# 0xMiden/miden-vm

Measured on NVIDIA H100. Metric: trace cells/sec proved, higher is better.
Workload: dtype u64

## Files before the change

### miden-vm_b200/csrc/kernels.cuh

```cuda
#pragma once
#include "gl.cuh"
#include <cuda_runtime.h>

namespace mk {
using gl::u64;
using gl::u32;
using gl::E2;

static constexpr u32 MAX_RANKS = 8;
struct PeerPtrs { u64* p[MAX_RANKS]; };
enum PushMode : u32 { PUSH_LOCAL = 0, PUSH_OWNER = 1, PUSH_ALL = 2 };
struct PushDst { PeerPtrs pp; u32 rank, world, mode, owner_shift; };
inline PushDst local_dst(u64* p) { PushDst d{}; d.pp.p[0] = p; d.rank = 0; d.world = 1; d.mode = PUSH_LOCAL; d.owner_shift = 0; return d; }

void launch_barrier(const PeerPtrs& flags, u32 rank, u32 world, u64 epoch, u32* err, cudaStream_t st);
void launch_push(const u64* src, const PeerPtrs& dst, u32 rank, u32 world, size_t n, cudaStream_t st);

struct NttTables {
    u32 n, n1, n2, lo_bits;
    const u64* tw_n1;
    const u64* twi_n1;
    const u64* twi_n2;
    const u64* w_lo;
    const u64* w_hi;
    const u64* wi_lo;
    const u64* wi_hi;
};
struct PremulTables {
    const u64* tab_b;
    const u64* tab_c;
};

void launch_transpose_rm_to_cm(const u64* src_rm, u64* dst_cm, u32 n_rows, u32 width, u32* d_bad_flag, cudaStream_t st);
void launch_transpose_slice_push(const u64* src_slice, const PeerPtrs& dst_cm, const PeerPtrs& bad, u32 world, u32 row0, u32 n_rows_slice,
                                 u32 n_rows_total, u32 width, cudaStream_t st);
void launch_ingest_cm(const u64* src_cm, u64* dst_cm, size_t n, u32* d_bad_flag, cudaStream_t st);

void launch_intt(u64* cols, size_t col_stride, u32 n_cols, const NttTables& T, cudaStream_t st);

struct FwdItem { const u64* src; u64* dst; u32 base; u32 pad; };
void launch_fwd_ntt(const FwdItem* d_items, u32 n_items, const NttTables& T, const PremulTables& Pm, cudaStream_t st);

struct LeafMat { const u64* base; u32 width; u32 pad; };
struct LeafArgs { LeafMat m[8]; int n_mats; };
void launch_leaf_hash(const LeafArgs& a, u32 log_n, u32 log_blowup, const u64* prev_states, u32 prev_log_n,
                      u64* states_out, const PushDst* dig, u32 t0, u32 nt, cudaStream_t st, int perm = 0);
void launch_compress_layer(const u64* children, u64* parents, size_t n_parents, cudaStream_t st, int perm = 0);
void launch_fri_leaf_hash(const u64* evals , size_t rows, u32 log_arity, const PushDst& digests,
                          u32 log_b, u32 t0, u32 nt, cudaStream_t st, int perm = 0);
void launch_poseidon2_batch(u64* states, size_t n, cudaStream_t st);
void launch_compress_top(u64* tree, u32 d_from, u32 lg, u32 rank, int hash_kind, cudaStream_t st);
void launch_leaf_hash_b3(const LeafArgs& a, u32 log_n, u32 log_blowup, const u64* prev_states, u32 prev_log_n,
                         u64* states_out, const PushDst* dig, u32 t0, u32 nt, cudaStream_t st);
void launch_compress_layer_b3(const u64* children, u64* parents, size_t n_parents, cudaStream_t st);
void launch_fri_leaf_hash_b3(const u64* evals, size_t rows, u32 log_arity, const PushDst& digests, u32 log_b, u32 t0, u32 nt, cudaStream_t st);
void launch_grind_b3(const u32* d_input_words, u32 n_words, u32 bits, u64 start, u64 count, u64* d_result, cudaStream_t st);
void launch_leaf_hash_kk(const LeafArgs& a, u32 log_n, u32 log_blowup, const u64* prev_states, u32 prev_log_n,
                         u64* states_out, const PushDst* dig, u32 t0, u32 nt, cudaStream_t st);
void launch_compress_layer_kk(const u64* children, u64* parents, size_t n_parents, cudaStream_t st);
void launch_fri_leaf_hash_kk(const u64* evals, size_t rows, u32 log_arity, const PushDst& digests, u32 log_b, u32 t0, u32 nt, cudaStream_t st);
void launch_grind_kk(const u64* d_input_words, u32 n_words, u32 bits, u64 start, u64 count, u64* d_result, cudaStream_t st);

struct AirDev {
    const u32* code;
    const u64* consts;
    const u64* periodic;
    u32 n_instr, n_slots;
    u32 uses_selectors;
    u32 log_max_period, n_periodic;
};
struct ConstraintArgs {
    const u64* main_lde; u32 main_width;
    const u64* aux_lde; u32 aux_width_base;
    const u64* prep_lde;
    u32 log_n, log_blowup;
    AirDev air;
    const u64* publics;
    const u64* challenges;
    const u64* aux_values;
    E2 alpha, beta;
    const u64* acc_in; u32 acc_in_log_n;
    u64* acc_out;
    const NttTables* T;
    u32 t0, nt;
};
int launch_constraints(const ConstraintArgs& a, cudaStream_t st);

struct LogupArgs {
    const u64* main_cm;
    const u64* prep_cm;
    u32 log_n, n_cols;
    AirDev prog;
    const u64* publics; const u64* challenges;
    u64* aux_cm;
    u64* totals;
    u32* bad_flag;
};
int launch_logup_rows(const LogupArgs& a, cudaStream_t st);
void launch_ef_exclusive_scan(const u64* totals, size_t n, u64* acc0, u64* acc1, u64* final2, u64* scratch, cudaStream_t st);
static constexpr u32 LOGUP_MAX_COLS = 16;

static constexpr u32 REG_MAX = 4, REG_BLOCK = 128;
struct RegisterArgs {
    const u64* main_cm;
    const u64* prep_cm;
    u32 log_n, n_regs;
    u32 col0;
    AirDev prog;
    const u64* publics; const u64* challenges;
    u64* aux_cm;
    u64* scratch;
    u32* bad_flag;
};
size_t register_scratch_words(u32 log_n, u32 n_regs);
int launch_register_columns(const RegisterArgs& a, cudaStream_t st);

struct CheckArgs {
    const u64* main_cm;
    const u64* aux_cm;
    const u64* prep_cm;
    u32 log_n;
    AirDev prog;
    const u64* publics; const u64* challenges; const u64* aux_values;
    size_t row0, n_rows;
    unsigned long long* first;
    unsigned long long* failing_rows;
    u32 probe_k; u64* probe_value;
};
int launch_check_rows(const CheckArgs& a, cudaStream_t st);

static constexpr u32 CENSUS_SHARED_K = 256;
struct CensusArgs {
    const u64* main_cm; const u64* aux_cm; const u64* prep_cm;
    u32 log_n;
    AirDev prog;
    const u64* publics; const u64* challenges; const u64* aux_values;
    u32 n_cons;
    u32 instance;
    u32* row_count;
    unsigned long long* tally;
    unsigned long long* failing_rows;
    const u64* offsets;
    u64 max_failures;
    u64* failures;
    const u64* probes; size_t n_probes;
};
int launch_census_rows(const CensusArgs& a, cudaStream_t st);
int launch_census_list(const CensusArgs& a, cudaStream_t st);
void launch_count_exclusive_scan(const u32* counts, size_t n, u64* offsets, u64* total, u64* scratch, cudaStream_t st);

struct BalanceTable {
    u64* keys;
    u64* sums;
    unsigned long long* count;
    unsigned long long* first;
    u64 mask;
};
static constexpr u32 BALANCE_BOUNDARY = 0x100;
__host__ __device__ inline u64 balance_key(u32 inst, u64 row, u32 k) { return ((u64)inst << 48) | (row << 24) | k; }
static constexpr u32 BALANCE_MUTEX_MAX = 1024;
struct BalanceArgs {
    const u64* main_cm; u32 log_n;
    const u64* prep_cm;
    AirDev prog;
    const u64* publics; const u64* challenges;
    u32 instance, mode;
    const u32* mutex_pos; const u32* mutex_group; const u32* mutex_site; u32 n_mutex;
    BalanceTable t;
    unsigned long long* counters;
    u64* mutex_out;
    u64* contrib_out;
};
int launch_balance_rows(const BalanceArgs& a, cudaStream_t st);
void launch_balance_boundary(const BalanceTable& t, const u64* triples, u32 n, cudaStream_t st);
void launch_balance_finish(const BalanceTable& t, unsigned long long* counters, u64* out, cudaStream_t st);
void launch_balance_compare(const BalanceTable& a, const BalanceTable& b, unsigned long long* words, cudaStream_t st);

struct LookupFoldArgs {
    const u64* main_cm; u32 log_n, n_cols;
    const u64* prep_cm;
    AirDev prog;
    const u64* publics; const u64* challenges;
    const u32* marks;
    const u64* aux_cm;
    E2 final;
    u64* folds_out; u32 folds_cm;
    size_t row0, n_rows;
    unsigned long long* first;
    unsigned long long* failing_rows;
    unsigned long long* zero_u;
    u32 probe_col; u64* probe;
};
int launch_fold_rows(const LookupFoldArgs& a, cudaStream_t st);

static constexpr u32 FOLD_RECORD_WORDS = 11;
struct FoldCensusArgs {
    const u64* main_cm; u32 log_n, n_cols;
    const u64* prep_cm;
    AirDev prog;
    const u64* publics; const u64* challenges;
    const u32* marks;
    const u64* aux_cm;
    E2 final;
    u32 instance;
    u32* row_count;
    unsigned long long* tally;
    unsigned long long* failing_rows;
    const u64* offsets;
    u64 max_failures;
    u64* failures;
    const u64* probes; size_t n_probes;
};
int launch_fold_census_rows(const FoldCensusArgs& a, cudaStream_t st);
int launch_fold_census_list(const FoldCensusArgs& a, cudaStream_t st);

void launch_pow_bitrev(E2 y, u32 n, u64* wvec, u64* scratch, size_t p0, size_t cnt, cudaStream_t st);
void launch_ood_dot(const u64* coef, size_t col_stride, u32 n_cols, u32 n, const u64* w0, const u64* w1,
                    u64* partial, u32 n_chunks, cudaStream_t st);
void launch_ood_reduce(const u64* partial, u32 n_cols, u32 n_chunks, u64* out , cudaStream_t st);

struct DeepMat { const u64* base; u32 width; u32 log_n; u32 alpha_off; u32 pad; };
struct DeepArgs {
    const DeepMat* m; int n_mats;
    u32 log_n_max, log_blowup;
    const u64* apow;
    u32 total_w;
    E2 z0, z1, fz0, fz1, beta;
    PushDst out;
    const NttTables* T;
    u32 t0, nt;
};
void launch_deep(const DeepArgs& a, cudaStream_t st);

void launch_fri_fold(const u64* evals, u32 log_dom, u32 log_arity, E2 beta, const PushDst& next, u32 log_b, u32 t0, u32 nt,
                     cudaStream_t st);

void launch_grind(const u64* d_state12, u32 in_len, u32 bits, u64 start, u64 count, u64* d_result ,
                  cudaStream_t st, int perm = 0);

void launch_compare(const u64* a, const u64* b, size_t n, u32* flag, cudaStream_t st);
void launch_gather(const u64* const* d_ptrs, u64* d_out, size_t n, cudaStream_t st);
void launch_gather_push(const u64* const* d_ptrs, const int* d_owner, const PeerPtrs& out, u32 rank, u32 world, size_t n, cudaStream_t st);

void launch_export_lde_bitrev_rm(const u64* lde, u32 log_n, u32 log_blowup, u32 width, u64* out_rm, cudaStream_t st);

void upload_constants();
unsigned long long launch_count();
void count_launch();
void reset_launch_count();

}
```

### miden-vm_b200/csrc/ntt2.cuh

```cuda
#pragma once
#include "poseidon2_fast2.cuh"
#include "kernels.cuh"
#include "tma.cuh"

namespace ntt2 {
using gl::u64;
using gl::u32;

#if defined(__CUDA_ARCH__) || defined(MDN_EMULATED)
#define NTT2_FOR(i, n) for (u32 i = threadIdx.x; i < (u32)(n); i += blockDim.x)
#define NTT2_SYNC() __syncthreads()
#else
#define NTT2_FOR(i, n) for (u32 i = 0; i < (u32)(n); i++)
#define NTT2_SYNC() ((void)0)
#endif

GL_HD u32 tile_off(u32 idx, u32 cc, u32 log_cols) {
    u32 o = (idx << log_cols) + cc;
    return log_cols ? o : o + (o >> 3);
}
GL_HD u32 tile_words(u32 m, u32 log_cols) {
    u32 n = 1u << (m + log_cols);
    return log_cols ? n + (n >> 4) : n + (n >> 3) + 1;
}
GL_HD u32 tw_off(u32 m, u32 log_cols) { return (tile_words(m, log_cols) + 1u) & ~1u; }
GL_HD size_t smem_words_contig_fwd(u32 n2) { return (size_t)tw_off(n2, 0) + ((size_t)1 << n2) + 2; }
GL_HD size_t smem_words_contig_inv(u32 n2) { return (size_t)tw_off(n2, 0) + ((size_t)1 << n2) / 2 + 4; }
GL_HD size_t smem_words_strided(u32 n1, u32 log_c) { return (size_t)tw_off(n1, log_c) + ((size_t)1 << n1) / 2 + 4; }

GL_HD u32 pad16(u32 o) { return o + (o >> 4); }
template <bool P16 = false>
GL_HD u32 chunk_off(u32 i) { return P16 ? pad16(i) : tile_off(i, 0, 0); }
template <bool P16 = false>
GL_HD void load_chunk(u64* x, const u64* src, u32 n) {
#if defined(__CUDA_ARCH__)
    if (n >= 2 && (((size_t)src) & 15) == 0) {
        const ulonglong2* s2 = reinterpret_cast<const ulonglong2*>(src);
        NTT2_FOR(i, n / 2) { ulonglong2 v = s2[i]; x[chunk_off<P16>(2 * i)] = v.x; x[chunk_off<P16>(2 * i + 1)] = v.y; }
        return;
    }
#endif
    NTT2_FOR(i, n) x[chunk_off<P16>(i)] = src[i];
}
template <bool P16 = false>
GL_HD void store_chunk_canon(u64* dst, const u64* x, u32 n) {
#if defined(__CUDA_ARCH__)
    if (n >= 2 && (((size_t)dst) & 15) == 0) {
        ulonglong2* d2 = reinterpret_cast<ulonglong2*>(dst);
        NTT2_FOR(i, n / 2) d2[i] = make_ulonglong2(glf::canon_cc(x[chunk_off<P16>(2 * i)]), glf::canon_cc(x[chunk_off<P16>(2 * i + 1)]));
        return;
    }
#endif
    NTT2_FOR(i, n) dst[i] = glf::canon_cc(x[chunk_off<P16>(i)]);
}

struct TableLoad { bool async; };
GL_HD TableLoad table_load(u64* dst, const u64* src, u32 words, u64* bar) {
#if defined(__CUDA_ARCH__)
    const u32 bytes = (words * 8u + 15u) & ~15u;
    if (words >= 64 && ((((size_t)src) | ((size_t)dst)) & 15) == 0) {
        if (threadIdx.x == 0) { tma::mbar_init(bar, 1); }
        __syncthreads();
        if (threadIdx.x == 0) { tma::expect_tx(bar, bytes); tma::bulk_g2s(dst, src, bytes, bar); }
        return TableLoad{true};
    }
#endif
    (void)bar;
    NTT2_FOR(i, words) dst[i] = src[i];
    return TableLoad{false};
}
GL_HD void table_wait(TableLoad t, u64* bar) {
#if defined(__CUDA_ARCH__)
    if (t.async) tma::wait(bar, 0);
#endif
    (void)t; (void)bar;
}

template <bool STAGED>
GL_HD u64 tw_at(const u64* tw, u32 m, u32 s, u32 j) { return STAGED ? tw[((1u << s) - 1u) + j] : tw[j << (m - 1 - s)]; }

template <int LOGR, bool STAGED, bool UNIT0>
GL_HD void dit_bfly(u64* v, const u64* tw, u32 m, u32 b, u32 lo) {
    constexpr int R = 1 << LOGR;
#pragma unroll
    for (int st = 0; st < LOGR; st++) {
#pragma unroll
        for (int k = 0; k < R; k++) {
            if (k & (1 << st)) continue;
            const u32 jj = (u32)(k & ((1 << st) - 1));
            u64 c;
            if (UNIT0 && jj == 0) c = glf::canon_cc(v[k + (1 << st)]);
            else c = glf::cmul(v[k + (1 << st)], tw_at<STAGED>(tw, m, b + st, lo + (jj << b)));
            u64 a = v[k];
            v[k] = glf::add_const(a, c);
            v[k + (1 << st)] = glf::csub(a, c);
        }
    }
}
template <int LOGR, bool STAGED, bool UNIT0>
GL_HD void dit_group(u64* x, const u64* tw, u32 m, u32 b, u32 log_cols, u32 g) {
    constexpr int R = 1 << LOGR;
    u32 cc = g & ((1u << log_cols) - 1), gg = g >> log_cols;
    u32 lo = gg & ((1u << b) - 1), hi = gg >> b;
    u32 base = (hi << (b + LOGR)) | lo;
    u64 v[R];
#pragma unroll
    for (int k = 0; k < R; k++) v[k] = x[tile_off(base + ((u32)k << b), cc, log_cols)];
    dit_bfly<LOGR, STAGED, UNIT0>(v, tw, m, b, lo);
#pragma unroll
    for (int k = 0; k < R; k++) x[tile_off(base + ((u32)k << b), cc, log_cols)] = v[k];
}
template <int LOGR, bool UNIT0>
GL_HD void dif_bfly(u64* v, const u64* tw, u32 m, u32 b, u32 lo) {
    constexpr int R = 1 << LOGR;
#pragma unroll
    for (int st = LOGR - 1; st >= 0; st--) {
#pragma unroll
        for (int k = 0; k < R; k++) {
            if (k & (1 << st)) continue;
            const u32 jj = (u32)(k & ((1 << st) - 1));
            u64 a = v[k], c = glf::canon_cc(v[k + (1 << st)]);
            v[k] = glf::add_const(a, c);
            u64 d = glf::csub(a, c);
            v[k + (1 << st)] = (UNIT0 && jj == 0) ? d : glf::mul(d, tw_at<false>(tw, m, b + st, lo + (jj << b)));
        }
    }
}
template <int LOGR, bool UNIT0>
GL_HD void dif_group(u64* x, const u64* tw, u32 m, u32 b, u32 log_cols, u32 g) {
    constexpr int R = 1 << LOGR;
    u32 cc = g & ((1u << log_cols) - 1), gg = g >> log_cols;
    u32 lo = gg & ((1u << b) - 1), hi = gg >> b;
    u32 base = (hi << (b + LOGR)) | lo;
    u64 v[R];
#pragma unroll
    for (int k = 0; k < R; k++) v[k] = x[tile_off(base + ((u32)k << b), cc, log_cols)];
    dif_bfly<LOGR, UNIT0>(v, tw, m, b, lo);
#pragma unroll
    for (int k = 0; k < R; k++) x[tile_off(base + ((u32)k << b), cc, log_cols)] = v[k];
}

template <int LOGR, bool STAGED, bool UNIT0>
GL_HD void dit_round(u64* x, const u64* tw, u32 m, u32 b, u32 log_cols) {
    NTT2_FOR(g, 1u << (m - LOGR + log_cols)) dit_group<LOGR, STAGED, UNIT0>(x, tw, m, b, log_cols, g);
    NTT2_SYNC();
}
template <int LOGR, bool UNIT0>
GL_HD void dif_round(u64* x, const u64* tw, u32 m, u32 b, u32 log_cols) {
    NTT2_FOR(g, 1u << (m - LOGR + log_cols)) dif_group<LOGR, UNIT0>(x, tw, m, b, log_cols, g);
    NTT2_SYNC();
}
template <bool STAGED>
GL_HD void smem_dit(u64* x, const u64* tw, u32 m, u32 log_cols) {
    u32 b = 0;
    while (b < m) {
        u32 left = m - b;
        if (left >= 3 && left != 4) {
            if (b == 0) dit_round<3, STAGED, !STAGED>(x, tw, m, b, log_cols); else dit_round<3, STAGED, false>(x, tw, m, b, log_cols);
            b += 3;
        } else if (left == 4 || left == 2) {
            if (b == 0) dit_round<2, STAGED, !STAGED>(x, tw, m, b, log_cols); else dit_round<2, STAGED, false>(x, tw, m, b, log_cols);
            b += 2;
        } else {
            if (b == 0) dit_round<1, STAGED, !STAGED>(x, tw, m, b, log_cols); else dit_round<1, STAGED, false>(x, tw, m, b, log_cols);
            b += 1;
        }
    }
}
GL_HD void smem_dif(u64* x, const u64* tw, u32 m, u32 log_cols) {
    u32 top = m;
    while (top > 0) {
        if (top >= 3 && top != 4) {
            if (top == 3) dif_round<3, true>(x, tw, m, 0, log_cols); else dif_round<3, false>(x, tw, m, top - 3, log_cols);
            top -= 3;
        } else if (top == 4 || top == 2) {
            if (top == 2) dif_round<2, true>(x, tw, m, 0, log_cols); else dif_round<2, false>(x, tw, m, top - 2, log_cols);
            top -= 2;
        } else {
            dif_round<1, true>(x, tw, m, 0, log_cols);
            top -= 1;
        }
    }
}

GL_HD constexpr int sched_rounds(int m) { return m == 8 ? 2 : 3; }
GL_HD constexpr int sched_radix(int m, int i) { return m == 9 ? 3 : (i < 2 && (m != 10 || i == 0)) ? 4 : 3; }
GL_HD constexpr int sched_span(int m, int i) { return i == 0 ? 0 : sched_span(m, i - 1) + sched_radix(m, i - 1); }
GL_HD constexpr int sched_log_elems(int m) { return m == 9 ? 3 : 4; }

template <int LOGR, int B, int LC>
GL_HD void tile_get(u64 (&v)[1 << LOGR], const u64* x, u32 base, u32 cc) {
#pragma unroll
    for (int k = 0; k < (1 << LOGR); k++) v[k] = x[pad16(((base + ((u32)k << B)) << LC) + cc)];
}
template <int LOGR, int B, int LC>
GL_HD void tile_put(u64* x, const u64 (&v)[1 << LOGR], u32 base, u32 cc) {
#pragma unroll
    for (int k = 0; k < (1 << LOGR); k++) x[pad16(((base + ((u32)k << B)) << LC) + cc)] = v[k];
}
template <bool STAGED, int M, int LC, int I, class Ld, class St>
GL_HD void dit_sched(u64* x, const u64* tw, TableLoad tl, u64* bar, const Ld& ld, const St& st) {
    constexpr int R = sched_radix(M, I), B = sched_span(M, I);
    constexpr bool FIRST = I == 0, LAST = I + 1 == sched_rounds(M);
    NTT2_FOR(g, 1u << (M + LC - R)) {
        const u32 cc = g & ((1u << LC) - 1), gg = g >> LC, lo = gg & ((1u << B) - 1);
        const u32 base = ((gg >> B) << (B + R)) | lo;
        u64 v[1 << R];
        if constexpr (FIRST) { ld(v, base, cc); table_wait(tl, bar); } else tile_get<R, B, LC>(v, x, base, cc);
        dit_bfly<R, STAGED, B == 0 && !STAGED>(v, tw, (u32)M, (u32)B, lo);
        if constexpr (LAST) st(v, base, cc); else tile_put<R, B, LC>(x, v, base, cc);
    }
    if constexpr (!LAST) {
        NTT2_SYNC();
        dit_sched<STAGED, M, LC, I + 1>(x, tw, tl, bar, ld, st);
    }
}
template <int M, int LC, int I, class Ld, class St>
GL_HD void dif_sched(u64* x, const u64* tw, TableLoad tl, u64* bar, const Ld& ld, const St& st) {
    constexpr int R = sched_radix(M, I), B = sched_span(M, I);
    constexpr bool FIRST = I + 1 == sched_rounds(M), LAST = I == 0;
    NTT2_FOR(g, 1u << (M + LC - R)) {
        const u32 cc = g & ((1u << LC) - 1), gg = g >> LC, lo = gg & ((1u << B) - 1);
        const u32 base = ((gg >> B) << (B + R)) | lo;
        u64 v[1 << R];
        if constexpr (FIRST) { ld(v, base, cc); table_wait(tl, bar); } else tile_get<R, B, LC>(v, x, base, cc);
        dif_bfly<R, B == 0>(v, tw, (u32)M, (u32)B, lo);
        if constexpr (LAST) st(v, base, cc); else tile_put<R, B, LC>(x, v, base, cc);
    }
    if constexpr (!LAST) {
        NTT2_SYNC();
        dif_sched<M, LC, I - 1>(x, tw, tl, bar, ld, st);
    }
}

GL_HD u64 w_pow(const u64* hi, const u64* lo, u32 lo_bits, u64 e) {
    return glf::mul(hi[e >> lo_bits], lo[e & ((1ull << lo_bits) - 1)]);
}

template <int N1C, int N2C> GL_HD constexpr int strided_log_c() { return N1C >= 12 ? 0 : (12 - N1C < N2C ? 12 - N1C : N2C); }

template <int N1C = -1, int N2C = -1>
GL_HD void intt_strided_block(u32 bx, u32 by, u64* sm, u64* cols, size_t col_stride, const mk::NttTables& T, u32 log_c_rt) {
    const u32 n1 = N1C >= 0 ? (u32)N1C : T.n1, n2 = N2C >= 0 ? (u32)N2C : T.n2;
    const u32 log_c = N1C >= 0 && N2C >= 0 ? (u32)strided_log_c<N1C, N2C>() : log_c_rt;
    u32 C = 1u << log_c, N1 = 1u << n1, N2 = 1u << n2;
    u64* x = sm; u64* tw = sm + tw_off(n1, log_c); u64* bar = tw + N1 / 2 + 2;
    u64* col = cols + (size_t)by * col_stride;
    u32 j2_0 = bx * C;
    TableLoad tl = table_load(tw, T.twi_n1, N1 / 2, bar);
    if constexpr (N1C >= 0 && N2C >= 0) {
        constexpr int LC = strided_log_c<N1C, N2C>(), NR = sched_rounds(N1C);
        constexpr int RF = sched_radix(N1C, NR - 1), BF = sched_span(N1C, NR - 1), RL = sched_radix(N1C, 0);
        static_assert(BF + RF == N1C, "the rounds cover the pass");
        if (!tl.async) NTT2_SYNC();
        auto ld = [&](u64 (&v)[1 << RF], u32 base, u32 cc) {
#pragma unroll
            for (int k = 0; k < (1 << RF); k++) v[k] = col[(size_t)(base + ((u32)k << BF)) * N2 + j2_0 + cc];
        };
        auto st = [&](u64 (&v)[1 << RL], u32 base, u32 cc) {
            const u32 j2 = j2_0 + cc;
#pragma unroll
            for (int k = 0; k < (1 << RL); k++) {
                const u32 slot = base + (u32)k;
                u64 f = w_pow(T.wi_hi, T.wi_lo, T.lo_bits, (u64)j2 * gl::bitrev32(slot, n1));
                col[(size_t)slot * N2 + j2] = glf::cmul(v[k], f);
            }
        };
        dif_sched<N1C, LC, NR - 1>(x, tw, tl, bar, ld, st);
    } else {
        NTT2_FOR(idx, N1 * C) {
            u32 j1 = idx >> log_c, cc = idx & (C - 1);
            x[tile_off(j1, cc, log_c)] = col[(size_t)j1 * N2 + j2_0 + cc];
        }
        table_wait(tl, bar);
        NTT2_SYNC();
        smem_dif(x, tw, n1, log_c);
        NTT2_FOR(idx, N1 * C) {
            u32 slot = idx >> log_c, cc = idx & (C - 1);
            u32 k1 = gl::bitrev32(slot, n1);
            u32 j2 = j2_0 + cc;
            u64 f = w_pow(T.wi_hi, T.wi_lo, T.lo_bits, (u64)j2 * k1);
            col[(size_t)slot * N2 + j2] = glf::cmul(x[tile_off(slot, cc, log_c)], f);
        }
    }
}
template <int N2C = -1>
GL_HD void intt_contig_block(u32 bx, u32 by, u64* sm, u64* cols, size_t col_stride, const mk::NttTables& T) {
    const u32 n2 = N2C >= 0 ? (u32)N2C : T.n2;
    u32 N2 = 1u << n2;
    u64* x = sm; u64* tw = sm + tw_off(n2, 0); u64* bar = tw + N2 / 2 + 2;
    u64* chunk = cols + (size_t)by * col_stride + (size_t)bx * N2;
    TableLoad tl = table_load(tw, T.twi_n2, N2 / 2, bar);
    if constexpr (N2C >= 0) {
        constexpr int NR = sched_rounds(N2C), RF = sched_radix(N2C, NR - 1), BF = sched_span(N2C, NR - 1), RL = sched_radix(N2C, 0);
        static_assert(BF + RF == N2C, "the rounds cover the pass");
        if (!tl.async) NTT2_SYNC();
        auto ld = [&](u64 (&v)[1 << RF], u32 base, u32) {
#pragma unroll
            for (int k = 0; k < (1 << RF); k++) v[k] = chunk[base + ((u32)k << BF)];
        };
        auto st = [&](u64 (&v)[1 << RL], u32 base, u32) { tile_put<RL, 0, 0>(x, v, base, 0); };
        dif_sched<N2C, 0, NR - 1>(x, tw, tl, bar, ld, st);
        NTT2_SYNC();
        store_chunk_canon<true>(chunk, x, N2);
    } else {
        load_chunk(x, chunk, N2);
        table_wait(tl, bar);
        NTT2_SYNC();
        smem_dif(x, tw, n2, 0);
        store_chunk_canon(chunk, x, N2);
    }
}
static constexpr u32 FWD_LANES = 128;
template <int N1C = -1, int N2C = -1>
GL_HD void fwd_contig_block(u32 bx, u32 by, u64* sm, const mk::FwdItem* items, const mk::NttTables& T, const mk::PremulTables& Pm) {
    const u32 n1 = N1C >= 0 ? (u32)N1C : T.n1, n2 = N2C >= 0 ? (u32)N2C : T.n2, n = N1C >= 0 && N2C >= 0 ? (u32)(N1C + N2C) : T.n;
    u32 N1 = 1u << n1, N2 = 1u << n2;
    u64* x = sm; u64* tw = sm + tw_off(n2, 0); u64* bar = tw + N2;
    mk::FwdItem it = items[by];
    u32 p_hi = bx;
    u32 j1 = gl::bitrev32(p_hi, n1);
    const u64* src = it.src + (size_t)p_hi * N2;
    u64* dst = it.dst + (size_t)p_hi * N2;
    u64 fb = Pm.tab_b[(size_t)it.base * N1 + j1];
    const u64* tc = Pm.tab_c + (size_t)it.base * N2;
    TableLoad tl = table_load(tw, tc, N2, bar);
    if constexpr (N1C >= 0 && N2C >= 0) {
        constexpr int NR = sched_rounds(N2C), RF = sched_radix(N2C, 0), RL = sched_radix(N2C, NR - 1), BL = sched_span(N2C, NR - 1);
        static_assert(BL + RL == N2C, "the rounds cover the pass");
        load_chunk<true>(x, src, N2);
        NTT2_SYNC();
        const u64 mask = ((u64)1 << n) - 1;
        const u64 step = w_pow(T.w_hi, T.w_lo, T.lo_bits, ((u64)j1 << BL) & mask);
        auto ld = [&](u64 (&v)[1 << RF], u32 base, u32) { tile_get<RF, 0, 0>(v, x, base, 0); };
        auto st = [&](u64 (&v)[1 << RL], u32 base, u32) {
            u64 f = glf::mul(fb, w_pow(T.w_hi, T.w_lo, T.lo_bits, ((u64)j1 * base) & mask));
#pragma unroll
            for (int k = 0; k < (1 << RL); k++) {
                dst[base + ((u32)k << BL)] = glf::cmul(v[k], f);
                if (k + 1 < (1 << RL)) f = glf::mul(f, step);
            }
        };
        dit_sched<true, N2C, 0, 0>(x, tw, tl, bar, ld, st);
    } else {
        load_chunk(x, src, N2);
        table_wait(tl, bar);
        NTT2_SYNC();
        smem_dit<true>(x, tw, n2, 0);
        u32 lanes = N2 < FWD_LANES ? N2 : FWD_LANES;
        NTT2_FOR(l, lanes) {
            u64 f = fb, step = 1;
            if (n1 > 0) {
                u64 mask = ((u64)1 << n) - 1;
                f = glf::mul(fb, w_pow(T.w_hi, T.w_lo, T.lo_bits, ((u64)j1 * l) & mask));
                step = w_pow(T.w_hi, T.w_lo, T.lo_bits, ((u64)j1 * lanes) & mask);
            }
            for (u32 k2 = l; k2 < N2; k2 += lanes) {
                dst[k2] = glf::cmul(x[tile_off(k2, 0, 0)], f);
                if (n1 > 0) f = glf::mul(f, step);
            }
        }
    }
}
template <int N1C = -1, int N2C = -1>
GL_HD void fwd_strided_block(u32 bx, u32 by, u64* sm, const mk::FwdItem* items, const mk::NttTables& T, u32 log_c_rt) {
    const u32 n1 = N1C >= 0 ? (u32)N1C : T.n1, n2 = N2C >= 0 ? (u32)N2C : T.n2;
    const u32 log_c = N1C >= 0 && N2C >= 0 ? (u32)strided_log_c<N1C, N2C>() : log_c_rt;
    u32 C = 1u << log_c, N1 = 1u << n1, N2 = 1u << n2;
    u64* x = sm; u64* tw = sm + tw_off(n1, log_c); u64* bar = tw + N1 / 2 + 2;
    u64* col = items[by].dst;
    u32 k2_0 = bx * C;
    TableLoad tl = table_load(tw, T.tw_n1, N1 / 2, bar);
    if constexpr (N1C >= 0 && N2C >= 0) {
        constexpr int LC = strided_log_c<N1C, N2C>(), NR = sched_rounds(N1C), RF = sched_radix(N1C, 0);
        constexpr int RL = sched_radix(N1C, NR - 1), BL = sched_span(N1C, NR - 1);
        static_assert(BL + RL == N1C, "the rounds cover the pass");
        if (!tl.async) NTT2_SYNC();
        auto ld = [&](u64 (&v)[1 << RF], u32 base, u32 cc) {
#pragma unroll
            for (int k = 0; k < (1 << RF); k++) v[k] = col[(size_t)(base + (u32)k) * N2 + k2_0 + cc];
        };
        auto st = [&](u64 (&v)[1 << RL], u32 base, u32 cc) {
#pragma unroll
            for (int k = 0; k < (1 << RL); k++) col[(size_t)(base + ((u32)k << BL)) * N2 + k2_0 + cc] = glf::canon_cc(v[k]);
        };
        dit_sched<false, N1C, LC, 0>(x, tw, tl, bar, ld, st);
    } else {
        NTT2_FOR(idx, N1 * C) {
            u32 p_hi = idx >> log_c, cc = idx & (C - 1);
            x[tile_off(p_hi, cc, log_c)] = col[(size_t)p_hi * N2 + k2_0 + cc];
        }
        table_wait(tl, bar);
        NTT2_SYNC();
        smem_dit<false>(x, tw, n1, log_c);
        NTT2_FOR(idx, N1 * C) {
            u32 k1 = idx >> log_c, cc = idx & (C - 1);
            col[(size_t)k1 * N2 + k2_0 + cc] = glf::canon_cc(x[tile_off(k1, cc, log_c)]);
        }
    }
}

}
```

### miden-vm_b200/csrc/ntt_tables.hpp

```cpp
#pragma once
#include "gl.cuh"
#include "kernels.cuh"
#include <vector>

namespace ntt_tables {
using gl::u64;
using gl::u32;

inline void split_n(u32 n, u32& n1, u32& n2) {
    if (n <= 11) { n1 = 0; n2 = n; }
    else { n1 = n / 2; n2 = n - n1; }
}
inline std::vector<u64> powers(u64 base, size_t count) {
    std::vector<u64> v(count);
    u64 x = 1;
    for (size_t i = 0; i < count; i++) { v[i] = x; x = gl::mul(x, base); }
    return v;
}

struct NttHost {
    u32 n, n1, n2, lo_bits;
    std::vector<u64> data;
    size_t o_tw1, o_twi1, o_twi2, o_lo, o_hi, o_ilo, o_ihi;
    mk::NttTables view(const u64* b) const {
        return mk::NttTables{n, n1, n2, lo_bits, b + o_tw1, b + o_twi1, b + o_twi2, b + o_lo, b + o_hi, b + o_ilo, b + o_ihi};
    }
};
inline NttHost build_ntt(u32 n) {
    NttHost h;
    h.n = n; split_n(n, h.n1, h.n2);
    h.lo_bits = (n + 1) / 2;
    u32 n1 = h.n1, n2 = h.n2, lo_bits = h.lo_bits;
    u64 w = gl::two_adic_generator(n), wi = gl::inv(w);
    auto push = [&](const std::vector<u64>& v) {
        if (h.data.size() & 1) h.data.push_back(0);
        size_t off = h.data.size(); h.data.insert(h.data.end(), v.begin(), v.end()); return off;
    };
    u64 w1 = gl::two_adic_generator(n1), w2 = gl::two_adic_generator(n2);
    h.o_tw1 = push(powers(w1, n1 ? (size_t)1 << (n1 - 1) : 1));
    h.o_twi1 = push(powers(gl::inv(w1), n1 ? (size_t)1 << (n1 - 1) : 1));
    h.o_twi2 = push(powers(gl::inv(w2), n2 ? (size_t)1 << (n2 - 1) : 1));
    h.o_lo = push(powers(w, (size_t)1 << lo_bits));
    h.o_hi = push(powers(gl::exp_pow2(w, lo_bits), (size_t)1 << (n - lo_bits)));
    h.o_ilo = push(powers(wi, (size_t)1 << lo_bits));
    h.o_ihi = push(powers(gl::exp_pow2(wi, lo_bits), (size_t)1 << (n - lo_bits)));
    return h;
}

struct PremulHost {
    u32 n_bases;
    std::vector<u64> data;
    size_t o_b, o_c;
    mk::PremulTables view(const u64* b) const { return mk::PremulTables{b + o_b, b + o_c}; }
};
inline PremulHost build_premul(const std::vector<u64>& bases, u32 n) {
    u32 n1, n2; split_n(n, n1, n2);
    size_t N1 = (size_t)1 << n1, N2 = (size_t)1 << n2, nb = bases.size();
    u64 n_inv = gl::inv((u64)1 << n);
    PremulHost h;
    h.n_bases = (u32)nb;
    h.o_b = 0; h.o_c = nb * N1;
    h.data.assign(nb * (N1 + N2), 0);
    for (size_t b = 0; b < nb; b++) {
        u64 g = bases[b], gN1 = gl::exp_pow2(g, n1);
        u64 x = n_inv;
        for (size_t j1 = 0; j1 < N1; j1++) { h.data[h.o_b + b * N1 + j1] = x; x = gl::mul(x, g); }
        u64* tc = &h.data[h.o_c + b * N2];
        for (u32 s = 0; s < n2; s++) {
            u64 shift = gl::exp_pow2(gN1, n2 - 1 - s), ws = gl::two_adic_generator(s + 1);
            u64 y = shift;
            for (size_t j = 0; j < ((size_t)1 << s); j++) { tc[(((size_t)1 << s) - 1) + j] = y; y = gl::mul(y, ws); }
        }
    }
    return h;
}

}
```

### miden-vm_b200/csrc/poseidon2_fast2.cuh

```cuda
#pragma once
#include "gl.cuh"
#include "poseidon2.cuh"

namespace glf {
using gl::u64;
using gl::u32;
typedef unsigned __int128 u128;

struct W { u64 lo; u32 hi; };

static constexpr u64 EPS = 0xFFFFFFFFull;

GL_HD void addc64(u64 a, u64 b, u64& r, u32& c) {
#ifdef __CUDA_ARCH__
    asm("add.cc.u64 %0, %2, %3;\n\taddc.u32 %1, 0, 0;" : "=l"(r), "=r"(c) : "l"(a), "l"(b));
#else
    u128 s = (u128)a + b; r = (u64)s; c = (u32)(s >> 64);
#endif
}
GL_HD void subb64(u64 a, u64 b, u64& r, u32& m) {
#ifdef __CUDA_ARCH__
    asm("sub.cc.u64 %0, %2, %3;\n\tsubc.u32 %1, 0, 0;" : "=l"(r), "=r"(m) : "l"(a), "l"(b));
#else
    r = a - b; m = a < b ? 0xFFFFFFFFu : 0u;
#endif
}
GL_HD u64 mul_eps(u32 a) {
#if defined(__CUDA_ARCH__)
    u64 m;
    asm("mul.wide.u32 %0, %1, %2;" : "=l"(m) : "r"(a), "r"(0xFFFFFFFFu));
    return m;
#else
    return (u64)a * 0xFFFFFFFFull;
#endif
}
GL_HD u64 fold(u32 c, u64 r) { return r + (u64)(0u - c); }

GL_HD u64 canon(u64 x) { return x >= gl::P ? x - gl::P : x; }

GL_HD u64 red128(u64 lo, u64 hi) {
    u32 x2 = (u32)hi, x3 = (u32)(hi >> 32);
    u64 t, r; u32 m, c;
    subb64(lo, (u64)x3, t, m);
    t -= (u64)m;
    addc64(t, mul_eps(x2), r, c);
    return fold(c, r);
}
GL_HD u64 mul(u64 a, u64 b) {
    u128 q = (u128)a * b;
    return red128((u64)q, (u64)(q >> 64));
}
GL_HD u64 sqr(u64 a) { return mul(a, a); }

GL_HD u64 add_const(u64 x, u64 k) {
    u64 r; u32 c;
    addc64(x, k, r, c);
    return fold(c, r);
}

GL_HD W wide(u64 x) { W w; w.lo = x; w.hi = 0; return w; }
GL_HD void wadd(W& w, u64 x) {
#ifdef __CUDA_ARCH__
    asm("add.cc.u64 %0, %0, %2;\n\taddc.u32 %1, %1, 0;" : "+l"(w.lo), "+r"(w.hi) : "l"(x));
#else
    u128 s = (u128)w.lo + x; w.lo = (u64)s; w.hi += (u32)(s >> 64);
#endif
}
GL_HD void wadd(W& w, W x) {
#ifdef __CUDA_ARCH__
    asm("add.cc.u64 %0, %0, %2;\n\taddc.u32 %1, %1, %3;" : "+l"(w.lo), "+r"(w.hi) : "l"(x.lo), "r"(x.hi));
#else
    u128 s = (u128)w.lo + x.lo; w.lo = (u64)s; w.hi += x.hi + (u32)(s >> 64);
#endif
}
GL_HD W wsum(u64 a, u64 b) {
    W w;
    addc64(a, b, w.lo, w.hi);
    return w;
}
GL_HD void wsub(W& w, W x) {
#ifdef __CUDA_ARCH__
    u64 lo; u32 hi;
    asm("sub.cc.u64 %0, %2, %3;\n\tsubc.u32 %1, %4, %5;" : "=l"(lo), "=r"(hi) : "l"(w.lo), "l"(x.lo), "r"(w.hi), "r"(x.hi));
    w.lo = lo; w.hi = hi;
#else
    u32 b = w.lo < x.lo ? 1u : 0u; w.lo -= x.lo; w.hi = w.hi - x.hi - b;
#endif
}
GL_HD W wshl(u64 x, int k) { W w; w.lo = x << k; w.hi = (u32)(x >> (64 - k)); return w; }
GL_HD W wtriple(u64 x) { W w = wshl(x, 1); wadd(w, x); return w; }
GL_HD u64 wred(W w) {
    u64 r; u32 c;
    addc64(w.lo, mul_eps(w.hi), r, c);
    return fold(c, r);
}
static constexpr u64 P8_LO = 0xFFFFFFF800000008ull;
static constexpr u32 P8_HI = 7u;

GL_HD u64 canon_cc(u64 r) {
    u64 t; u32 m;
    subb64(r, gl::P, t, m);
    return t - (u64)m;
}
GL_HD u64 csub(u64 a, u64 b) {
    u64 d; u32 m;
    subb64(a, b, d, m);
    return d - (u64)m;
}
GL_HD u64 cadd(u64 a, u64 b) { return csub(a, gl::P - b); }
GL_HD u64 cmul(u64 a, u64 b) { return canon_cc(mul(a, b)); }

GL_HD u64 half(u64 x) { return (x >> 1) + (u64)((u32)x & 1u) * 0x7FFFFFFF80000001ull; }
template <int K>
GL_HD u64 div2k(u64 x) {
    u32 n = (0u - (u32)x) & ((1u << K) - 1u);
    u64 q = (x >> K) + (n ? 1ull : 0ull);
    return (u64)(n << (32 - K)) * EPS + q;
}

GL_HD W wshl96(W w, int k) { W r; r.lo = w.lo << k; r.hi = (w.hi << k) | (u32)(w.lo >> (64 - k)); return r; }
GL_HD W wshr96(W w, int k) { W r; r.lo = (w.lo >> k) | ((u64)w.hi << (64 - k)); r.hi = w.hi >> k; return r; }
GL_HD W whalf(W w) {
    wadd(w, gl::P & (0ull - (w.lo & 1ull)));
    return wshr96(w, 1);
}
template <int K>
GL_HD W wdiv2k(W w) {
    u32 n = (0u - (u32)w.lo) & ((1u << K) - 1u);
    w.hi += n;
    wsub(w, wide((u64)n * EPS));
    return wshr96(w, K);
}

struct Acc160 { u64 lo, mid; u32 hi; };
GL_HD void acc_mul(Acc160& A, u64 x, u64 y) {
    u128 q = (u128)x * y;
    u64 ql = (u64)q, qh = (u64)(q >> 64);
#if defined(__CUDA_ARCH__)
    asm("add.cc.u64 %0, %0, %3;\n\taddc.cc.u64 %1, %1, %4;\n\taddc.u32 %2, %2, 0;" : "+l"(A.lo), "+l"(A.mid), "+r"(A.hi) : "l"(ql), "l"(qh));
#else
    u128 s0 = (u128)A.lo + ql;
    u128 s1 = (u128)A.mid + qh + (u64)(s0 >> 64);
    A.lo = (u64)s0; A.mid = (u64)s1; A.hi += (u32)(s1 >> 64);
#endif
}
GL_HD u64 acc_reduce(const Acc160& A) {
    u64 r = canon_cc(red128(A.lo, A.mid));
    return csub(r, (u64)A.hi << 32);
}

}

namespace p2f {
using gl::u64;
using gl::u32;
using glf::W;

#if !defined(__CUDA_ARCH__) && defined(P2F_TRACK_BOUNDS)
static u32 p2f_max_hi = 0;
#endif

GL_HD u64 sbox(u64 x) {
    u64 x2 = glf::sqr(x), x3 = glf::mul(x2, x), x4 = glf::sqr(x2);
    return glf::mul(x3, x4);
}

GL_HD void external_layer(u64* s) {
    W y[12];
#pragma unroll
    for (int c = 0; c < 12; c += 4) {
        W t01 = glf::wsum(s[c], s[c + 1]), t23 = glf::wsum(s[c + 2], s[c + 3]);
        W t0123 = t01; glf::wadd(t0123, t23);
        W t01123 = t0123; glf::wadd(t01123, s[c + 1]);
        W t01233 = t0123; glf::wadd(t01233, s[c + 3]);
        W y3 = t01233; glf::wadd(y3, glf::wshl(s[c], 1));
        W y1 = t01123; glf::wadd(y1, glf::wshl(s[c + 2], 1));
        glf::wadd(t01123, t01);
        glf::wadd(t01233, t23);
        y[c] = t01123; y[c + 1] = y1; y[c + 2] = t01233; y[c + 3] = y3;
    }
#pragma unroll
    for (int l = 0; l < 4; l++) {
        W col = y[l];
        glf::wadd(col, y[4 + l]); glf::wadd(col, y[8 + l]);
#pragma unroll
        for (int c = 0; c < 12; c += 4) {
            W o = y[c + l];
            glf::wadd(o, col);
            s[c + l] = glf::wred(o);
        }
    }
}

#define P2F_OFF_LO {0xfffffffb00000005ull, 0xffffffbb00000045ull, 0xfffffbfb00000405ull, 0xffffc3bb00003c45ull, \
                    0xfffc77fb00038805ull, 0xffcb07bb0034f845ull, 0xfce573fb031a8c05ull, 0xd171cbbb2e8e3445ull}
#define P2F_OFF_HI {0x4u, 0x44u, 0x404u, 0x3c44u, 0x38804u, 0x34f844u, 0x31a8c04u, 0x2e8e3444u}
static const u64 H_OFF_LO[8] = P2F_OFF_LO;
static const u32 H_OFF_HI[8] = P2F_OFF_HI;
#ifdef __CUDACC__
__constant__ u64 D_OFF_LO[8] = P2F_OFF_LO;
__constant__ u32 D_OFF_HI[8] = P2F_OFF_HI;
#endif

GL_HD void internal_rounds_lazy(u64* s, const u64* rc) {
#ifdef __CUDA_ARCH__
    const u64* off_lo = D_OFF_LO; const u32* off_hi = D_OFF_HI;
#else
    const u64* off_lo = H_OFF_LO; const u32* off_hi = H_OFF_HI;
#endif
    W L[11];
#pragma unroll
    for (int i = 0; i < 11; i++) L[i] = glf::wide(s[i + 1]);
    u64 s0 = s[0];
    int r = 0;
#pragma unroll 1
    for (int blk = 0; blk < 3; blk++) {
        const int n = blk < 2 ? 8 : 6;
#pragma unroll 1
        for (int j = 0; j < n; j++, r++) {
            s0 = sbox(glf::add_const(s0, rc[r]));
            W sum = glf::wide(s0);
#pragma unroll
            for (int i = 0; i < 11; i++) glf::wadd(sum, L[i]);
            W sump = sum;
            { W off; off.lo = off_lo[j]; off.hi = off_hi[j]; glf::wadd(sump, off); }
            W t;
            t = sump; glf::wsub(t, glf::wshl(s0, 1)); s0 = glf::wred(t);
            glf::wadd(L[0], sum);
            L[1] = glf::wshl96(L[1], 1); glf::wadd(L[1], sum);
            L[2] = glf::whalf(L[2]); glf::wadd(L[2], sum);
            t = glf::wshl96(L[3], 1); glf::wadd(t, L[3]); glf::wadd(t, sum); L[3] = t;
            L[4] = glf::wshl96(L[4], 2); glf::wadd(L[4], sum);
            t = sump; glf::wsub(t, glf::whalf(L[5])); L[5] = t;
            { W t3 = glf::wshl96(L[6], 1); glf::wadd(t3, L[6]); t = sump; glf::wsub(t, t3); L[6] = t; }
            t = sump; glf::wsub(t, glf::wshl96(L[7], 2)); L[7] = t;
            L[8] = glf::wdiv2k<2>(L[8]); glf::wadd(L[8], sum);
            t = sump; glf::wsub(t, glf::wdiv2k<2>(L[9])); L[9] = t;
            L[10] = glf::wdiv2k<3>(L[10]); glf::wadd(L[10], sum);
#if !defined(__CUDA_ARCH__) && defined(P2F_TRACK_BOUNDS)
            for (int i = 0; i < 11; i++) if (L[i].hi > p2f_max_hi) p2f_max_hi = L[i].hi;
#endif
        }
#pragma unroll
        for (int i = 0; i < 11; i++) L[i] = glf::wide(glf::wred(L[i]));
    }
    s[0] = s0;
#pragma unroll
    for (int i = 0; i < 11; i++) s[i + 1] = L[i].lo;
}

#ifdef __CUDA_ARCH__
#define P2F_RC_EXT_INITIAL p2::D_RC_EXT_INITIAL
#define P2F_RC_EXT_TERMINAL p2::D_RC_EXT_TERMINAL
#define P2F_RC_INTERNAL p2::D_RC_INTERNAL
#else
#define P2F_RC_EXT_INITIAL p2::P2_RC_EXT_INITIAL
#define P2F_RC_EXT_TERMINAL p2::P2_RC_EXT_TERMINAL
#define P2F_RC_INTERNAL p2::P2_RC_INTERNAL
#endif

GL_HD void permute(u64* s) {
    external_layer(s);
#pragma unroll 1
    for (int phase = 0; phase < 2; phase++) {
        const u64* rc = phase ? P2F_RC_EXT_TERMINAL : P2F_RC_EXT_INITIAL;
#pragma unroll 1
        for (int r = 0; r < 4; r++) {
#pragma unroll
            for (int i = 0; i < 12; i++) s[i] = sbox(glf::add_const(s[i], rc[12 * r + i]));
            external_layer(s);
        }
        if (phase == 0) internal_rounds_lazy(s, P2F_RC_INTERNAL);
    }
}

}
```

Baseline: 597.7 million.

## Use power-of-two twiddles in first NTT radix round and fold coset premul into load

In the Goldilocks field, 8th roots of unity are powers of two, so the first radix-8 round (b==0) replaces its twiddle multiplications with shift-and-reduce operations (mul_pow2/shl_red). The forward contiguous pass now loads the shared n2 twiddle table (half size) instead of per-base staged tables, and moves the per-element tab_c scaling into the chunk load as a multiply. The tab_c table is rebuilt as bit-reversed powers of gN1. The aim is fewer full modular multiplies and less shared memory in butterflies, at the cost of an extra multiply per element on load and more code complexity in the shift reductions.

```diff
diff --git a/miden-vm_b200/csrc/kernels.cuh b/miden-vm_b200/csrc/kernels.cuh
--- a/miden-vm_b200/csrc/kernels.cuh
+++ b/miden-vm_b200/csrc/kernels.cuh
@@ -20,6 +20,7 @@
     u32 n, n1, n2, lo_bits;
     const u64* tw_n1;
     const u64* twi_n1;
+    const u64* tw_n2;
     const u64* twi_n2;
     const u64* w_lo;
     const u64* w_hi;
diff --git a/miden-vm_b200/csrc/ntt2.cuh b/miden-vm_b200/csrc/ntt2.cuh
--- a/miden-vm_b200/csrc/ntt2.cuh
+++ b/miden-vm_b200/csrc/ntt2.cuh
@@ -24,7 +24,7 @@
     return log_cols ? n + (n >> 4) : n + (n >> 3) + 1;
 }
 GL_HD u32 tw_off(u32 m, u32 log_cols) { return (tile_words(m, log_cols) + 1u) & ~1u; }
-GL_HD size_t smem_words_contig_fwd(u32 n2) { return (size_t)tw_off(n2, 0) + ((size_t)1 << n2) + 2; }
+GL_HD size_t smem_words_contig_fwd(u32 n2) { return (size_t)tw_off(n2, 0) + ((size_t)1 << n2) / 2 + 4; }
 GL_HD size_t smem_words_contig_inv(u32 n2) { return (size_t)tw_off(n2, 0) + ((size_t)1 << n2) / 2 + 4; }
 GL_HD size_t smem_words_strided(u32 n1, u32 log_c) { return (size_t)tw_off(n1, log_c) + ((size_t)1 << n1) / 2 + 4; }
 
@@ -43,6 +43,21 @@
     NTT2_FOR(i, n) x[chunk_off<P16>(i)] = src[i];
 }
 template <bool P16 = false>
+GL_HD void load_chunk_mul(u64* x, const u64* src, const u64* f, u32 n) {
+#if defined(__CUDA_ARCH__)
+    if (n >= 2 && ((((size_t)src) | ((size_t)f)) & 15) == 0) {
+        const ulonglong2* s2 = reinterpret_cast<const ulonglong2*>(src);
+        const ulonglong2* f2 = reinterpret_cast<const ulonglong2*>(f);
+        NTT2_FOR(i, n / 2) {
+            ulonglong2 v = s2[i], w = f2[i];
+            x[chunk_off<P16>(2 * i)] = glf::mul(v.x, w.x); x[chunk_off<P16>(2 * i + 1)] = glf::mul(v.y, w.y);
+        }
+        return;
+    }
+#endif
+    NTT2_FOR(i, n) x[chunk_off<P16>(i)] = glf::mul(src[i], f[i]);
+}
+template <bool P16 = false>
 GL_HD void store_chunk_canon(u64* dst, const u64* x, u32 n) {
 #if defined(__CUDA_ARCH__)
     if (n >= 2 && (((size_t)dst) & 15) == 0) {
@@ -76,10 +91,10 @@
     (void)t; (void)bar;
 }
 
-template <bool STAGED>
-GL_HD u64 tw_at(const u64* tw, u32 m, u32 s, u32 j) { return STAGED ? tw[((1u << s) - 1u) + j] : tw[j << (m - 1 - s)]; }
-
-template <int LOGR, bool STAGED, bool UNIT0>
+GL_HD u64 tw_at(const u64* tw, u32 m, u32 s, u32 j) { return tw[j << (m - 1 - s)]; }
+GL_HD constexpr int tw_log2(bool inv, int s, int j) { return (int)(((inv ? 153u : 39u) * ((u32)j << (5 - s))) % 192u); }
+
+template <int LOGR, bool POW2>
 GL_HD void dit_bfly(u64* v, const u64* tw, u32 m, u32 b, u32 lo) {
     constexpr int R = 1 << LOGR;
 #pragma unroll
@@ -88,16 +103,21 @@
         for (int k = 0; k < R; k++) {
             if (k & (1 << st)) continue;
             const u32 jj = (u32)(k & ((1 << st) - 1));
-            u64 c;
-            if (UNIT0 && jj == 0) c = glf::canon_cc(v[k + (1 << st)]);
-            else c = glf::cmul(v[k + (1 << st)], tw_at<STAGED>(tw, m, b + st, lo + (jj << b)));
             u64 a = v[k];
-            v[k] = glf::add_const(a, c);
-            v[k + (1 << st)] = glf::csub(a, c);
-        }
-    }
-}
-template <int LOGR, bool STAGED, bool UNIT0>
+            if (POW2) {
+                const int e = tw_log2(false, st, (int)jj);
+                const u64 c = glf::mul_pow2(v[k + (1 << st)], e % 96);
+                v[k] = e < 96 ? glf::add_const(a, c) : glf::csub(a, c);
+                v[k + (1 << st)] = e < 96 ? glf::csub(a, c) : glf::add_const(a, c);
+            } else {
+                const u64 c = glf::cmul(v[k + (1 << st)], tw_at(tw, m, b + st, lo + (jj << b)));
+                v[k] = glf::add_const(a, c);
+                v[k + (1 << st)] = glf::csub(a, c);
+            }
+        }
+    }
+}
+template <int LOGR, bool POW2>
 GL_HD void dit_group(u64* x, const u64* tw, u32 m, u32 b, u32 log_cols, u32 g) {
     constexpr int R = 1 << LOGR;
     u32 cc = g & ((1u << log_cols) - 1), gg = g >> log_cols;
@@ -106,11 +126,11 @@
     u64 v[R];
 #pragma unroll
     for (int k = 0; k < R; k++) v[k] = x[tile_off(base + ((u32)k << b), cc, log_cols)];
-    dit_bfly<LOGR, STAGED, UNIT0>(v, tw, m, b, lo);
+    dit_bfly<LOGR, POW2>(v, tw, m, b, lo);
 #pragma unroll
     for (int k = 0; k < R; k++) x[tile_off(base + ((u32)k << b), cc, log_cols)] = v[k];
 }
-template <int LOGR, bool UNIT0>
+template <int LOGR, bool POW2>
 GL_HD void dif_bfly(u64* v, const u64* tw, u32 m, u32 b, u32 lo) {
     constexpr int R = 1 << LOGR;
 #pragma unroll
@@ -122,11 +142,16 @@
             u64 a = v[k], c = glf::canon_cc(v[k + (1 << st)]);
             v[k] = glf::add_const(a, c);
             u64 d = glf::csub(a, c);
-            v[k + (1 << st)] = (UNIT0 && jj == 0) ? d : glf::mul(d, tw_at<false>(tw, m, b + st, lo + (jj << b)));
-        }
-    }
-}
-template <int LOGR, bool UNIT0>
+            if (POW2) {
+                const int e = tw_log2(true, st, (int)jj);
+                v[k + (1 << st)] = e < 96 ? glf::shl_red(d, e) : gl::P - glf::canon_cc(glf::shl_red(d, e - 96));
+            } else {
+                v[k + (1 << st)] = glf::mul(d, tw_at(tw, m, b + st, lo + (jj << b)));
+            }
+        }
+    }
+}
+template <int LOGR, bool POW2>
 GL_HD void dif_group(u64* x, const u64* tw, u32 m, u32 b, u32 log_cols, u32 g) {
     constexpr int R = 1 << LOGR;
     u32 cc = g & ((1u << log_cols) - 1), gg = g >> log_cols;
@@ -135,34 +160,33 @@
     u64 v[R];
 #pragma unroll
     for (int k = 0; k < R; k++) v[k] = x[tile_off(base + ((u32)k << b), cc, log_cols)];
-    dif_bfly<LOGR, UNIT0>(v, tw, m, b, lo);
+    dif_bfly<LOGR, POW2>(v, tw, m, b, lo);
 #pragma unroll
     for (int k = 0; k < R; k++) x[tile_off(base + ((u32)k << b), cc, log_cols)] = v[k];
 }
 
-template <int LOGR, bool STAGED, bool UNIT0>
+template <int LOGR, bool POW2>
 GL_HD void dit_round(u64* x, const u64* tw, u32 m, u32 b, u32 log_cols) {
-    NTT2_FOR(g, 1u << (m - LOGR + log_cols)) dit_group<LOGR, STAGED, UNIT0>(x, tw, m, b, log_cols, g);
+    NTT2_FOR(g, 1u << (m - LOGR + log_cols)) dit_group<LOGR, POW2>(x, tw, m, b, log_cols, g);
     NTT2_SYNC();
 }
-template <int LOGR, bool UNIT0>
+template <int LOGR, bool POW2>
 GL_HD void dif_round(u64* x, const u64* tw, u32 m, u32 b, u32 log_cols) {
-    NTT2_FOR(g, 1u << (m - LOGR + log_cols)) dif_group<LOGR, UNIT0>(x, tw, m, b, log_cols, g);
+    NTT2_FOR(g, 1u << (m - LOGR + log_cols)) dif_group<LOGR, POW2>(x, tw, m, b, log_cols, g);
     NTT2_SYNC();
 }
-template <bool STAGED>
 GL_HD void smem_dit(u64* x, const u64* tw, u32 m, u32 log_cols) {
     u32 b = 0;
     while (b < m) {
         u32 left = m - b;
         if (left >= 3 && left != 4) {
-            if (b == 0) dit_round<3, STAGED, !STAGED>(x, tw, m, b, log_cols); else dit_round<3, STAGED, false>(x, tw, m, b, log_cols);
+            if (b == 0) dit_round<3, true>(x, tw, m, b, log_cols); else dit_round<3, false>(x, tw, m, b, log_cols);
             b += 3;
         } else if (left == 4 || left == 2) {
-            if (b == 0) dit_round<2, STAGED, !STAGED>(x, tw, m, b, log_cols); else dit_round<2, STAGED, false>(x, tw, m, b, log_cols);
+            if (b == 0) dit_round<2, true>(x, tw, m, b, log_cols); else dit_round<2, false>(x, tw, m, b, log_cols);
             b += 2;
         } else {
-            if (b == 0) dit_round<1, STAGED, !STAGED>(x, tw, m, b, log_cols); else dit_round<1, STAGED, false>(x, tw, m, b, log_cols);
+            if (b == 0) dit_round<1, true>(x, tw, m, b, log_cols); else dit_round<1, false>(x, tw, m, b, log_cols);
             b += 1;
         }
     }
@@ -198,7 +222,7 @@
 #pragma unroll
     for (int k = 0; k < (1 << LOGR); k++) x[pad16(((base + ((u32)k << B)) << LC) + cc)] = v[k];
 }
-template <bool STAGED, int M, int LC, int I, class Ld, class St>
+template <int M, int LC, int I, class Ld, class St>
 GL_HD void dit_sched(u64* x, const u64* tw, TableLoad tl, u64* bar, const Ld& ld, const St& st) {
     constexpr int R = sched_radix(M, I), B = sched_span(M, I);
     constexpr bool FIRST = I == 0, LAST = I + 1 == sched_rounds(M);
@@ -207,12 +231,12 @@
         const u32 base = ((gg >> B) << (B + R)) | lo;
         u64 v[1 << R];
         if constexpr (FIRST) { ld(v, base, cc); table_wait(tl, bar); } else tile_get<R, B, LC>(v, x, base, cc);
-        dit_bfly<R, STAGED, B == 0 && !STAGED>(v, tw, (u32)M, (u32)B, lo);
+        dit_bfly<R, B == 0>(v, tw, (u32)M, (u32)B, lo);
         if constexpr (LAST) st(v, base, cc); else tile_put<R, B, LC>(x, v, base, cc);
     }
     if constexpr (!LAST) {
         NTT2_SYNC();
-        dit_sched<STAGED, M, LC, I + 1>(x, tw, tl, bar, ld, st);
+        dit_sched<M, LC, I + 1>(x, tw, tl, bar, ld, st);
     }
 }
 template <int M, int LC, int I, class Ld, class St>
@@ -316,7 +340,7 @@
 GL_HD void fwd_contig_block(u32 bx, u32 by, u64* sm, const mk::FwdItem* items, const mk::NttTables& T, const mk::PremulTables& Pm) {
     const u32 n1 = N1C >= 0 ? (u32)N1C : T.n1, n2 = N2C >= 0 ? (u32)N2C : T.n2, n = N1C >= 0 && N2C >= 0 ? (u32)(N1C + N2C) : T.n;
     u32 N1 = 1u << n1, N2 = 1u << n2;
-    u64* x = sm; u64* tw = sm + tw_off(n2, 0); u64* bar = tw + N2;
+    u64* x = sm; u64* tw = sm + tw_off(n2, 0); u64* bar = tw + N2 / 2 + 2;
     mk::FwdItem it = items[by];
     u32 p_hi = bx;
     u32 j1 = gl::bitrev32(p_hi, n1);
@@ -324,11 +348,11 @@
     u64* dst = it.dst + (size_t)p_hi * N2;
     u64 fb = Pm.tab_b[(size_t)it.base * N1 + j1];
     const u64* tc = Pm.tab_c + (size_t)it.base * N2;
-    TableLoad tl = table_load(tw, tc, N2, bar);
+    TableLoad tl = table_load(tw, T.tw_n2, N2 / 2, bar);
     if constexpr (N1C >= 0 && N2C >= 0) {
         constexpr int NR = sched_rounds(N2C), RF = sched_radix(N2C, 0), RL = sched_radix(N2C, NR - 1), BL = sched_span(N2C, NR - 1);
         static_assert(BL + RL == N2C, "the rounds cover the pass");
-        load_chunk<true>(x, src, N2);
+        load_chunk_mul<true>(x, src, tc, N2);
         NTT2_SYNC();
         const u64 mask = ((u64)1 << n) - 1;
         const u64 step = w_pow(T.w_hi, T.w_lo, T.lo_bits, ((u64)j1 << BL) & mask);
@@ -341,12 +365,12 @@
                 if (k + 1 < (1 << RL)) f = glf::mul(f, step);
             }
         };
-        dit_sched<true, N2C, 0, 0>(x, tw, tl, bar, ld, st);
+        dit_sched<N2C, 0, 0>(x, tw, tl, bar, ld, st);
     } else {
-        load_chunk(x, src, N2);
+        load_chunk_mul(x, src, tc, N2);
         table_wait(tl, bar);
         NTT2_SYNC();
-        smem_dit<true>(x, tw, n2, 0);
+        smem_dit(x, tw, n2, 0);
         u32 lanes = N2 < FWD_LANES ? N2 : FWD_LANES;
         NTT2_FOR(l, lanes) {
             u64 f = fb, step = 1;
@@ -384,7 +408,7 @@
 #pragma unroll
             for (int k = 0; k < (1 << RL); k++) col[(size_t)(base + ((u32)k << BL)) * N2 + k2_0 + cc] = glf::canon_cc(v[k]);
         };
-        dit_sched<false, N1C, LC, 0>(x, tw, tl, bar, ld, st);
+        dit_sched<N1C, LC, 0>(x, tw, tl, bar, ld, st);
     } else {
         NTT2_FOR(idx, N1 * C) {
             u32 p_hi = idx >> log_c, cc = idx & (C - 1);
@@ -392,7 +416,7 @@
         }
         table_wait(tl, bar);
         NTT2_SYNC();
-        smem_dit<false>(x, tw, n1, log_c);
+        smem_dit(x, tw, n1, log_c);
         NTT2_FOR(idx, N1 * C) {
             u32 k1 = idx >> log_c, cc = idx & (C - 1);
             col[(size_t)k1 * N2 + k2_0 + cc] = glf::canon_cc(x[tile_off(k1, cc, log_c)]);
diff --git a/miden-vm_b200/csrc/ntt_tables.hpp b/miden-vm_b200/csrc/ntt_tables.hpp
--- a/miden-vm_b200/csrc/ntt_tables.hpp
+++ b/miden-vm_b200/csrc/ntt_tables.hpp
@@ -21,9 +21,9 @@
 struct NttHost {
     u32 n, n1, n2, lo_bits;
     std::vector<u64> data;
-    size_t o_tw1, o_twi1, o_twi2, o_lo, o_hi, o_ilo, o_ihi;
+    size_t o_tw1, o_twi1, o_tw2, o_twi2, o_lo, o_hi, o_ilo, o_ihi;
     mk::NttTables view(const u64* b) const {
-        return mk::NttTables{n, n1, n2, lo_bits, b + o_tw1, b + o_twi1, b + o_twi2, b + o_lo, b + o_hi, b + o_ilo, b + o_ihi};
+        return mk::NttTables{n, n1, n2, lo_bits, b + o_tw1, b + o_twi1, b + o_tw2, b + o_twi2, b + o_lo, b + o_hi, b + o_ilo, b + o_ihi};
     }
 };
 inline NttHost build_ntt(u32 n) {
@@ -39,6 +39,7 @@
     u64 w1 = gl::two_adic_generator(n1), w2 = gl::two_adic_generator(n2);
     h.o_tw1 = push(powers(w1, n1 ? (size_t)1 << (n1 - 1) : 1));
     h.o_twi1 = push(powers(gl::inv(w1), n1 ? (size_t)1 << (n1 - 1) : 1));
+    h.o_tw2 = push(powers(w2, n2 ? (size_t)1 << (n2 - 1) : 1));
     h.o_twi2 = push(powers(gl::inv(w2), n2 ? (size_t)1 << (n2 - 1) : 1));
     h.o_lo = push(powers(w, (size_t)1 << lo_bits));
     h.o_hi = push(powers(gl::exp_pow2(w, lo_bits), (size_t)1 << (n - lo_bits)));
@@ -66,11 +67,8 @@
         u64 x = n_inv;
         for (size_t j1 = 0; j1 < N1; j1++) { h.data[h.o_b + b * N1 + j1] = x; x = gl::mul(x, g); }
         u64* tc = &h.data[h.o_c + b * N2];
-        for (u32 s = 0; s < n2; s++) {
-            u64 shift = gl::exp_pow2(gN1, n2 - 1 - s), ws = gl::two_adic_generator(s + 1);
-            u64 y = shift;
-            for (size_t j = 0; j < ((size_t)1 << s); j++) { tc[(((size_t)1 << s) - 1) + j] = y; y = gl::mul(y, ws); }
-        }
+        x = 1;
+        for (size_t j2 = 0; j2 < N2; j2++) { tc[gl::bitrev32((u32)j2, n2)] = x; x = gl::mul(x, gN1); }
     }
     return h;
 }
diff --git a/miden-vm_b200/csrc/poseidon2_fast2.cuh b/miden-vm_b200/csrc/poseidon2_fast2.cuh
--- a/miden-vm_b200/csrc/poseidon2_fast2.cuh
+++ b/miden-vm_b200/csrc/poseidon2_fast2.cuh
@@ -109,6 +109,17 @@
 }
 GL_HD u64 cadd(u64 a, u64 b) { return csub(a, gl::P - b); }
 GL_HD u64 cmul(u64 a, u64 b) { return canon_cc(mul(a, b)); }
+
+GL_HD u64 shl_red(u64 x, int e) {
+    if (e >= 64) { x = red128(x << (e - 32), x >> (96 - e)); e = 32; }
+    if (e == 0) return x;
+    if (e <= 32) return wred(wshl(x, e));
+    return red128(x << e, x >> (64 - e));
+}
+GL_HD u64 mul_pow2(u64 x, int e) {
+    if (e < 96) return canon_cc(shl_red(x, e));
+    return canon_cc(gl::P - canon_cc(shl_red(x, e - 96)));
+}
 
 GL_HD u64 half(u64 x) { return (x >> 1) + (u64)((u32)x & 1u) * 0x7FFFFFFF80000001ull; }
 template <int K>
```

Result: no change. 599.6 million, median of 6 (+0.3%).
